# SumitTarafder/Figbird

Hardware: AMD Instinct MI355X
Metric: gaps/sec (+ filled-bases/sec), synthetic 1e5-gap set recipe, jump-library fill pass (higher is better)
Workload: dtype f64

## Files before the change

figbird_amd/api.py:

```python
from __future__ import annotations

import ctypes as C
import os
from dataclasses import dataclass
from dataclasses import replace as dc_replace
from typing import List, Optional

import numpy as np

from . import build as _build

c_double_p = C.POINTER(C.c_double)
c_i32_p = C.POINTER(C.c_int32)
c_i64_p = C.POINTER(C.c_int64)
c_u8_p = C.POINTER(C.c_uint8)


class FigModel(C.Structure):
    _fields_ = [
        ("max_read_length", C.c_int32), ("error_pos_dist", c_double_p), ("in_pos_dist", c_double_p),
        ("del_pos_dist", c_double_p), ("error_type_probs", C.c_double * 25),
        ("insert_len_dist_smoothed", c_double_p), ("max_insert_size", C.c_int32),
        ("insert_threshold_min", C.c_int32), ("insert_threshold_max", C.c_int32), ("gap_prob_cutoff", C.c_int32),
        ("partial_flag", C.c_int32), ("unmapped_flag", C.c_int32), ("script_itr", C.c_int32),
# ... 42 lines not shown

class FigReadPlacement(C.Structure):
    _fields_ = [("ll_drawn", c_double_p), ("ll_other", c_double_p), ("sum_other", c_double_p), ("off_other", c_i32_p), ("n_valid", c_i32_p),
                ("pq", c_u8_p), ("state", c_u8_p)]


PLACE_OFF, PLACE_ON, PLACE_NONE, PLACE_MAX_PQ = 0, 1, 255, 60


@dataclass
class Placement:
    ll_drawn: np.ndarray
    ll_other: np.ndarray
    sum_other: np.ndarray
    off_other: np.ndarray
    n_valid: np.ndarray
    pq: np.ndarray
    state: np.ndarray


class FigStats(C.Structure):
    _fields_ = [("kernel_ms", C.c_double), ("h2d_ms", C.c_double), ("d2h_ms", C.c_double),
                ("packed_bytes", C.c_int64), ("place_calls", C.c_int64), ("alg_flops", C.c_double),
                ("n_launches", C.c_int32), ("pad0", C.c_int32), ("spec_flops", C.c_double),
                ("mle_alg_flops", C.c_double), ("mle_exec_flops", C.c_double)]


EXPORTS = ["fig_version", "fig_strerror", "fig_ctx_create", "fig_ctx_destroy", "fig_ctx_set_model",
           "fig_results_capacity", "fig_batch_upload", "fig_fill_resident", "fig_fill_resident_ex", "fig_batch_free", "fig_fill_gaps",
           "fig_get_stats", "fig_batch_probe_reach", "fig_batch_set_ot_preset", "fig_batch_quality", "fig_batch_placement"]

_lib = None
_host = None


def load_library(path: Optional[str] = None) -> C.CDLL:
    global _lib
    if _lib is not None and path is None:
        return _lib
    p = path or _build.LIB
    if not os.path.exists(p):
        raise RuntimeError(f"libfighip.so not built at {p}: run `python -m figbird_amd.build` (there is no CPU fallback)")
    lib = C.CDLL(p)
    lib.fig_version.restype = C.c_int
    lib.fig_strerror.restype = C.c_char_p
    lib.fig_strerror.argtypes = [C.c_int]
    lib.fig_ctx_create.argtypes = [C.c_int, C.POINTER(C.c_void_p)]
# ... 474 lines not shown
```

figbird_amd/csrc/fig_abi.hip:

```cpp
#include <hip/hip_runtime.h>

#include <algorithm>
#include <cstdio>
#include <cstdlib>
#include <cstring>
#include <new>
#include <vector>
#include <chrono>
#include <thread>
#include <mutex>

#include "../../include/figbird_hip.h"
#include "fig_engine.h"
#include "fig_pack.h"
#include "fig_abi_host.h"
#include "fig_quality.h"
#include "fig_quality_host.h"
#include "fig_placement.h"

#ifdef FIG_PROF
#define FIG_PROF_BEGIN() const unsigned long long _k0 = __builtin_readcyclecounter()
#define FIG_PROF_FLUSH() do { if (E.lane == 0) { atomicAdd(&B.counters[FIG_CNT_WAIT], E.wait_cycles); atomicAdd(&B.counters[FIG_CNT_WAVE], (unsigned long long)__builtin_readcyclecounter() - _k0); \
    for (int i = 0; i < FIG_PROF_SLOTS; i++) if (E.prof[i]) atomicAdd(&B.counters[i < FIG_PROF_SPLIT ? FIG_CNT_PROF_LO + i : FIG_CNT_PROF_HI + (i - FIG_PROF_SPLIT)], E.prof[i]); } } while (0)
#else
// ... 49 lines not shown
    FigEng E; FigScr work;
    fig_kernel_begin(E, M, B, A, LDS_TAB, work);
    FIG_PROF_BEGIN();
    fig_pop_loop(E, B, A, [&] { return fig_src_order(B, A); }, [&](int gi) { fig_item_fill<LDS_TAB>(E, work, gi); });
    FIG_PROF_FLUSH();
    fig_kernel_flush(E, B);
}

template <bool LDS_TAB, int NT>
__global__ void __launch_bounds__(NT, (NT <= 256 ? 2 : 1)) fig_begin_kernel(FigDevModel M, FigDevBatch B, FigKernArgs A) {
    FigEng E; FigScr work;
    fig_kernel_begin(E, M, B, A, LDS_TAB, work);
    fig_pop_loop(E, B, A, [&] { return fig_src_order(B, A); }, [&](int gi) { fig_item_begin<LDS_TAB>(E, work, gi); });
    fig_kernel_flush(E, B);
}

template <bool LDS_TAB, int NT>
__global__ void __launch_bounds__(NT, (NT <= 256 ? 2 : 1)) fig_probe_kernel(FigDevModel M, FigDevBatch B, FigKernArgs A) {
    FigEng E; FigScr work;
    fig_kernel_begin(E, M, B, A, LDS_TAB, work);
    fig_pop_loop(E, B, A, [&] { return fig_src_order(B, A); }, [&](int gi) { fig_item_probe<LDS_TAB>(E, work, gi); });
}

static_assert(sizeof(FigItem) == sizeof(int4) && sizeof(FigEntry) == sizeof(int4), "item records travel as int4");
template <bool LDS_TAB, int NT>
__global__ void __launch_bounds__(NT, (NT <= 256 ? 2 : 1)) fig_eval_kernel(FigDevModel M, FigDevBatch B, FigKernArgs A, const int4 *items, int n_items) {
    FigEng E; FigScr work;
    fig_kernel_begin(E, M, B, A, LDS_TAB, work);
    FIG_PROF_BEGIN();
    fig_pop_loop(E, B, A, [&] { return FigItemSrc<FigItem>{(const FigItem *)items, 0, n_items}; }, [&](FigItem it) { fig_item_eval<LDS_TAB>(E, work, it); });
    FIG_PROF_FLUSH();
    fig_kernel_flush(E, B);
}

__global__ void __launch_bounds__(64) fig_replay_kernel(FigDevModel M, FigDevBatch B, const int4 *entries, int n) {
    if ((int)blockIdx.x >= n) return;
    FigEng E{}; FigScr work{};
    fig_eng_ident(E, threadIdx.x, blockDim.x, 64);
    E.M = &M; E.B = &B; E.nteams = 1; E.S = (FigState *)fig_lds;
    const FigEntry en = ((const FigEntry *)entries)[blockIdx.x];
    fig_item_replay(E, work, en);
}

template <bool LDS_TAB, int NT>
__global__ void __launch_bounds__(NT, (NT <= 256 ? 2 : 1)) fig_end_kernel(FigDevModel M, FigDevBatch B, FigKernArgs A, const int *list, int n) {
    FigEng E; FigScr work;
    fig_kernel_begin(E, M, B, A, LDS_TAB, work);
    fig_pop_loop(E, B, A, [&] { return FigItemSrc<int>{list, 0, n}; }, [&](int gi) { fig_item_end<LDS_TAB>(E, work, gi); });
    fig_kernel_flush(E, B);
}

__global__ void __launch_bounds__(256) fig_stream_kernel(FigDevModel M, FigDevBatch B, uint32_t *out) {
    for (long long gi = blockIdx.x; gi < B.n_gaps; gi += gridDim.x) {
        const FigDevGap &g = B.gaps[gi];
        const int L = M.L;
        const long long n = (long long)((g.nU + FIG_SH_C - 1) / FIG_SH_C) * L * (FIG_SH_C / 2);
        for (long long i = threadIdx.x; i < n; i += blockDim.x) {
            const int sp = (int)(i % (FIG_SH_C / 2));
            const long long cj = i / (FIG_SH_C / 2);
            const int j = (int)(cj % L);
            uint32_t v = 0;
            for (int h = 0; h < 2; h++) {
                const long long r = (cj / L) * FIG_SH_C + 2 * sp + h;
// ... 4 lines not shown
                    if (len == L && !(aux & 2)) {
                        const uint32_t w = B.packed[B.u.woff[idx] + (j >> 4)];
                        e = 0x1000u | (2u * (4u * (unsigned)(aux & 1) + ((w >> ((j & 15) * 2)) & 3u)));
                    }
                }
                v |= e << (16 * h);
            }
            out[g.streamOff + i] = v;
        }
    }
}

#define FIG_HIP(call) do { hipError_t _e = (call); if (_e != hipSuccess) { ctx->last_hip = (int)_e; return FIG_EHIP; } } while (0)

struct DevBuf { void *p = nullptr; };

struct FigTmpBufs {
    std::vector<void *> bufs;
    ~FigTmpBufs() { for (void *p : bufs) hipFree(p); }
    void *alloc(size_t n) { void *p = nullptr; if (hipMalloc(&p, n ? n : 8) != hipSuccess) return nullptr; bufs.push_back(p); return p; }
};

struct FigLane { hipStream_t stream = nullptr; hipEvent_t done = nullptr; int32_t *queue_head = nullptr; uint8_t *scratch = nullptr; FigItem *d_items = nullptr; FigEntry *d_entries = nullptr; size_t cap = 0;
                 FigGapCtl *h_ctl = nullptr; FigItem *h_items = nullptr; FigEntry *h_entries = nullptr; int qsel = 0; };

struct fig_ctx {
    int device = 0;
    hipStream_t stream = nullptr;
    hipEvent_t ev0 = nullptr, ev1 = nullptr;
    int n_cu = 0;
    int last_hip = 0;
    bool have_model = false;
    FigDevModel dm;
    DevBuf d_model_tabs;
    fig_model hm;
    bool have_batch = false;
    FigDevBatch db;
    std::vector<int32_t> h_order;
    struct Cls { FigLaunchClass c; int blocks; int capacity; };
    std::vector<Cls> classes;
    std::vector<DevBuf> bufs;
    int64_t n_gaps = 0, n_ureads = 0, n_preads = 0, str_total = 0;
    std::vector<int64_t> h_str_off;
    int nslots = 32;
    std::vector<FigLane> lanes;
    fig_stats stats;
    int sh_on = FIG_SH_SC;
    std::vector<uint8_t> h_ot;
    uint8_t *d_ot = nullptr;
};

static int dev_alloc(fig_ctx *ctx, size_t bytes, void **out) {
    DevBuf b;
    if (bytes == 0) bytes = 8;
    hipError_t e = hipMalloc(&b.p, bytes);
    if (e != hipSuccess) { ctx->last_hip = (int)e; return FIG_ENOMEM; }
    ctx->bufs.push_back(b);
    *out = b.p;
    return FIG_OK;
}

template <typename T>
static int dev_upload(fig_ctx *ctx, const std::vector<T> &v, const T **out) {
    void *p = nullptr;
    int rc = dev_alloc(ctx, v.size() * sizeof(T), &p);
    if (rc) return rc;
    if (!v.empty()) {
        hipError_t e = hipMemcpyAsync(p, v.data(), v.size() * sizeof(T), hipMemcpyHostToDevice, ctx->stream);
        if (e != hipSuccess) { ctx->last_hip = (int)e; return FIG_EHIP; }
    }
// ... 71 lines not shown
    if (hipMemcpy(ctx->d_model_tabs.p, all.data(), all.size() * sizeof(double), hipMemcpyHostToDevice) != hipSuccess) return FIG_EHIP;
    fig_model_point(ctx->dm, o, (const double *)ctx->d_model_tabs.p);
    ctx->have_model = true;
    return FIG_OK;
}

extern "C" int64_t fig_results_capacity(const fig_model *m, const fig_gap_batch *b) {
    if (!m || !b) return FIG_EINVAL;
    return fig_pack_results_capacity(m, b);
}

enum FigKind { FIG_K_FILL, FIG_K_BEGIN, FIG_K_EVAL, FIG_K_END, FIG_K_PROBE };

template <typename... P, typename... Args>
static hipError_t launch_one(void (*k)(P...), size_t lds, int nt, int blocks, hipStream_t stream, Args... args) {
    hipError_t e = hipFuncSetAttribute((const void *)k, hipFuncAttributeMaxDynamicSharedMemorySize, (int)lds);
    if (e != hipSuccess) return e;
    hipLaunchKernelGGL(k, dim3(blocks), dim3(nt), lds, stream, args...);
    return hipGetLastError();
}

template <bool LDS_TAB, int NT>
static hipError_t launch_kind(fig_ctx *ctx, const fig_ctx::Cls &c, const FigDevBatch &db, hipStream_t stream, FigKind kind, int blocks, const void *list, int n, int qsel) {
    const FigKernArgs A = fig_kargs_of(c.c, qsel, ctx->sh_on);
    switch (kind) {
        case FIG_K_FILL: return launch_one(fig_fill_kernel<LDS_TAB, NT>, c.c.lds, NT, blocks, stream, ctx->dm, db, A);
        case FIG_K_BEGIN: return launch_one(fig_begin_kernel<LDS_TAB, NT>, c.c.lds, NT, blocks, stream, ctx->dm, db, A);
        case FIG_K_PROBE: return launch_one(fig_probe_kernel<LDS_TAB, NT>, c.c.lds, NT, blocks, stream, ctx->dm, db, A);
        case FIG_K_EVAL: return launch_one(fig_eval_kernel<LDS_TAB, NT>, c.c.lds, NT, blocks, stream, ctx->dm, db, A, (const int4 *)list, n);
        case FIG_K_END: return launch_one(fig_end_kernel<LDS_TAB, NT>, c.c.lds, NT, blocks, stream, ctx->dm, db, A, (const int *)list, n);
    }
    return hipErrorInvalidValue;
}

static hipError_t launch_any(fig_ctx *ctx, const fig_ctx::Cls &c, const FigDevBatch &db, hipStream_t stream, FigKind kind, int blocks, const void *list, int n, int qsel = 0) {
    if (c.c.tiles > 0) return launch_kind<true, 512>(ctx, c, db, stream, kind, blocks, list, n, qsel);
    if (c.c.lds_tab) return c.c.nt == 256 ? launch_kind<true, 256>(ctx, c, db, stream, kind, blocks, list, n, qsel) : launch_kind<true, 512>(ctx, c, db, stream, kind, blocks, list, n, qsel);
    return launch_kind<false, 512>(ctx, c, db, stream, kind, blocks, list, n, qsel);
}

extern "C" int fig_batch_upload(fig_ctx *ctx, const fig_gap_batch *b) {
    if (!ctx || !b) return FIG_EINVAL;
    if (!ctx->have_model) return FIG_EINVAL;
    hipSetDevice(ctx->device);
    free_batch(ctx);
    const fig_model *m = &ctx->hm;
    hipEventRecord(ctx->ev0, ctx->stream);
// ... 30 lines not shown
    UP(p_pos, p.pos); UP(p_aux, p.aux); UP(p_clip, p.clip); UP(p_ref, p.refpos); UP(p_len, p.len); UP(p_woff, p.woff); UP(p_qoff, p.qoff);
#undef UP
    db.u.clip = nullptr; db.u.refpos = nullptr; db.u.qoff = nullptr;
    void *p;
    if (m->unmapped_flag) {
        if ((rc = dev_alloc(ctx, (size_t)K.stream_total * 4, &p))) return rc;
        db.ustream = (const uint32_t *)p;
        FIG_HIP(hipMemsetD32Async((hipDeviceptr_t)p, (int)(((0x1000u | FIG_SH_ONE) << 16) | (0x1000u | FIG_SH_ONE)), (size_t)K.stream_total, ctx->stream));
        if (ng > 0) {
            hipLaunchKernelGGL(fig_stream_kernel, dim3((unsigned)std::min<int64_t>(ng, 4096)), dim3(256), 0, ctx->stream, ctx->dm, db, (uint32_t *)p);
            FIG_HIP(hipGetLastError());
        }
    }
    if ((rc = dev_alloc(ctx, (size_t)ng * 4, &p))) return rc; db.filled_len = (int32_t *)p;
    if ((rc = dev_alloc(ctx, (size_t)ng * 4, &p))) return rc; db.gaptofill = (int32_t *)p;
    if ((rc = dev_alloc(ctx, (size_t)K.str_total, &p))) return rc; db.str = (char *)p;
    if ((rc = dev_alloc(ctx, 64 * (ctx->classes.size() + 1), &p))) return rc; db.queue_head = (int32_t *)p;
    if ((rc = dev_alloc(ctx, FIG_CNT_N * sizeof(unsigned long long), &p))) return rc; db.counters = (unsigned long long *)p;
    size_t total_blocks = 0;
    for (const fig_ctx::Cls &c : ctx->classes) total_blocks += (size_t)c.capacity;
    if ((rc = dev_alloc(ctx, (size_t)stride * std::max<size_t>(total_blocks, 1), &p))) return rc; db.scratch = (uint8_t *)p;
    if ((rc = dev_alloc(ctx, (size_t)K.persist_total + 256, &p))) return rc; db.persist = (uint8_t *)p;
    if ((rc = dev_alloc(ctx, (size_t)std::max<int64_t>(ng, 1) * sizeof(FigGapCtl), &p))) return rc; db.gapctl = (FigGapCtl *)p;
    if ((rc = dev_alloc(ctx, (size_t)std::max<int64_t>(ng, 1), &p))) return rc; ctx->d_ot = (uint8_t *)p; db.ot_preset = ctx->d_ot;
    ctx->h_ot = K.ot_preset;
    FIG_HIP(hipMemcpyAsync(ctx->d_ot, ctx->h_ot.data(), (size_t)std::max<int64_t>(ng, 1), hipMemcpyHostToDevice, ctx->stream));
    ctx->nslots = K.nslots;
    {   size_t blk = 0;
        for (size_t ci = 0; ci < ctx->classes.size(); ci++) {
            const fig_ctx::Cls &c = ctx->classes[ci];
            ctx->lanes.push_back(FigLane());
            FigLane &l = ctx->lanes.back();
            if (hipStreamCreate(&l.stream) != hipSuccess || hipEventCreateWithFlags(&l.done, hipEventDisableTiming) != hipSuccess) return FIG_EHIP;
            l.queue_head = db.queue_head + 16 * (ci + 1);
            l.scratch = db.scratch + (size_t)stride * blk; blk += (size_t)c.capacity;
            l.cap = (size_t)std::max(c.c.q_end - c.c.q_begin, 1) * (size_t)(K.nslots + 1);
            if ((rc = dev_alloc(ctx, l.cap * sizeof(FigItem), &p))) return rc; l.d_items = (FigItem *)p;
            if ((rc = dev_alloc(ctx, l.cap * sizeof(FigEntry), &p))) return rc; l.d_entries = (FigEntry *)p;
            if (hipHostMalloc((void **)&l.h_ctl, (size_t)std::max<int64_t>(ng, 1) * sizeof(FigGapCtl), hipHostMallocDefault) != hipSuccess) return FIG_ENOMEM;
            if (hipHostMalloc((void **)&l.h_items, l.cap * sizeof(FigItem), hipHostMallocDefault) != hipSuccess) return FIG_ENOMEM;
            if (hipHostMalloc((void **)&l.h_entries, l.cap * sizeof(FigEntry), hipHostMallocDefault) != hipSuccess) return FIG_ENOMEM;
        }
    }
    db.scratch_stride = stride;
    db.capG = K.capG; db.capR = K.capR; db.capP = K.capP; db.capC = K.capC; db.capW = K.capW; db.capE = K.capE;
    db.n_ureads = ctx->n_ureads;
    FIG_HIP(hipMemsetAsync(db.counters, 0, FIG_CNT_N * sizeof(unsigned long long), ctx->stream));
    FIG_HIP(hipMemsetAsync(db.queue_head, 0, 64 * (ctx->classes.size() + 1), ctx->stream));
    hipEventRecord(ctx->ev1, ctx->stream);
    FIG_HIP(hipStreamSynchronize(ctx->stream));
    float ms = 0; hipEventElapsedTime(&ms, ctx->ev0, ctx->ev1);
    ctx->stats.h2d_ms = ms;
    ctx->stats.packed_bytes = K.packed_bytes();
    ctx->have_batch = true;
    if (!K.ot_given && m->partial_flag && ng > 0 && (rc = fig_ot_carry_measured(ctx, ng))) { free_batch(ctx); return rc; }
    return FIG_OK;
}

extern "C" int fig_batch_probe_reach(fig_ctx *ctx, uint8_t *reach) {
    if (!ctx || !reach || !ctx->have_batch) return FIG_EINVAL;
    hipSetDevice(ctx->device);
// ... 6 lines not shown
    for (const fig_ctx::Cls &c : ctx->classes) {
        FIG_HIP(hipMemsetAsync(db.queue_head, 0, 8, ctx->stream));
        FIG_HIP(launch_any(ctx, c, db, ctx->stream, FIG_K_PROBE, c.blocks, nullptr, 0));
    }
    std::vector<FigGapCtl> ctl((size_t)ng);
    FIG_HIP(hipMemcpyAsync(ctl.data(), db.gapctl, (size_t)ng * sizeof(FigGapCtl), hipMemcpyDeviceToHost, ctx->stream));
    FIG_HIP(hipStreamSynchronize(ctx->stream));
    for (int64_t g = 0; g < ng; g++) reach[g] = ctl[g].reach ? 1 : 0;
    return FIG_OK;
}

extern "C" int fig_batch_set_ot_preset(fig_ctx *ctx, const uint8_t *preset) {
    if (!ctx || !preset || !ctx->have_batch) return FIG_EINVAL;
    hipSetDevice(ctx->device);
    const int64_t ng = ctx->n_gaps;
    for (int64_t g = 0; g < ng; g++) ctx->h_ot[(size_t)g] = preset[g] ? 1 : 0;
    if (ng > 0) { FIG_HIP(hipMemcpy(ctx->d_ot, ctx->h_ot.data(), (size_t)ng, hipMemcpyHostToDevice)); }
    return FIG_OK;
}

static int run_class_parallel(fig_ctx *ctx, const fig_ctx::Cls &c, FigLane &ln, const FigKnobs &knobs) {
    FigDevBatch db = ctx->db;
    db.queue_head = ln.queue_head; db.scratch = ln.scratch;
    hipStream_t stream = ln.stream;
    hipSetDevice(ctx->device);
    int nl = 0;
    hipError_t e;
    auto fail = [&](hipError_t er) { ctx->last_hip = (int)er; return -1; };
    const int capacity = std::max(1, c.capacity);
    auto launch = [&](FigKind kind, int n_work, const void *list) {
        hipError_t er = launch_any(ctx, c, db, stream, kind, std::min(capacity, n_work), list, n_work, ln.qsel);
        ln.qsel ^= 1; nl++;
        return er;
    };
    if ((e = launch(FIG_K_BEGIN, c.c.q_end - c.c.q_begin, nullptr)) != hipSuccess) return fail(e);
    FigGapCtl *ctl = ln.h_ctl;
    const size_t ctl_bytes = (size_t)ctx->n_gaps * sizeof(FigGapCtl);
    const std::vector<int> ids(ctx->h_order.begin() + c.c.q_begin, ctx->h_order.begin() + c.c.q_end);
    FigRound R;
    auto now = [] { return std::chrono::duration<double, std::milli>(std::chrono::steady_clock::now().time_since_epoch()).count(); };
    const double t_start = now();
    double t_prev = now(); int round = 0, last_items = 0, last_active = 0, last_chunk = 0, n_active_max = 0;
    while (true) {
        if ((e = hipMemcpyAsync(ctl, db.gapctl, ctl_bytes, hipMemcpyDeviceToHost, stream)) != hipSuccess) return fail(e);
        if ((e = hipStreamSynchronize(stream)) != hipSuccess) return fail(e);
        fig_plan_round(ids, ctl, capacity, c.c.nsplit, ctx->nslots, knobs.minc, knobs.ipw, n_active_max, R);
        if (knobs.log) { double t = now(); fprintf(stderr, "[figsched] capG=%d round %d: active=%d chunk=%d items=%d blocks=%d  %.1f ms\n", c.c.capG, round, last_active, last_chunk, last_items, capacity, t - t_prev); t_prev = t; }
        round++;
        if (R.n_active == 0) break;
        if (ln.cap < R.items.size() || ln.cap < R.entries.size()) return fail(hipErrorOutOfMemory);
        const int n_items = (int)R.items.size(), n_ent = (int)R.entries.size();
        const size_t items_bytes = R.items.size() * sizeof(FigItem), ent_bytes = R.entries.size() * sizeof(FigEntry);
        last_items = n_items; last_active = R.n_active; last_chunk = R.chunk;
        if (n_items > 0) {
            memcpy(ln.h_items, R.items.data(), items_bytes);
            if ((e = hipMemcpyAsync(ln.d_items, ln.h_items, items_bytes, hipMemcpyHostToDevice, stream)) != hipSuccess) return fail(e);
            if ((e = launch(FIG_K_EVAL, n_items, ln.d_items)) != hipSuccess) return fail(e);
        }
        memcpy(ln.h_entries, R.entries.data(), ent_bytes);
        if ((e = hipMemcpyAsync(ln.d_entries, ln.h_entries, ent_bytes, hipMemcpyHostToDevice, stream)) != hipSuccess) return fail(e);
        hipLaunchKernelGGL(fig_replay_kernel, dim3(n_ent), dim3(64), sizeof(FigState) + 64, stream, ctx->dm, db, (const int4 *)ln.d_entries, n_ent);
        if ((e = hipGetLastError()) != hipSuccess) return fail(e);
        nl++;
    }
    std::vector<int> endlist;
    for (int g : ids) if (ctl[g].status == FIG_GAP_LOOP_DONE) endlist.push_back(g);
    if (!endlist.empty()) {
        if ((e = hipStreamSynchronize(stream)) != hipSuccess) return fail(e);
        memcpy(ln.h_items, endlist.data(), endlist.size() * sizeof(int));
        if ((e = hipMemcpyAsync(ln.d_items, ln.h_items, endlist.size() * sizeof(int), hipMemcpyHostToDevice, stream)) != hipSuccess) return fail(e);
        if ((e = launch(FIG_K_END, (int)endlist.size(), ln.d_items)) != hipSuccess) return fail(e);
        if (knobs.log) { const double t0 = now(); hipStreamSynchronize(stream); fprintf(stderr, "[figsched] capG=%d end kernel: %d gaps, %.1f ms (lane done at %.1f ms since its first round)\n", c.c.capG, (int)endlist.size(), now() - t0, now() - t_start); }
    }
    return nl;
}

extern "C" int fig_fill_resident(fig_ctx *ctx, fig_gap_results *out) { return fig_fill_resident_ex(ctx, out, nullptr); }

extern "C" int fig_fill_resident_ex(fig_ctx *ctx, fig_gap_results *out, const fig_gap_support *sup) {
    if (!ctx || !out || !ctx->have_batch) return FIG_EINVAL;
    if (!out->filled_len || !out->gaptofill || !out->str_off || (!out->str && ctx->str_total > 0)) return FIG_EINVAL;
    if (sup && (!sup->counts || !sup->origin)) return FIG_EINVAL;
    hipSetDevice(ctx->device);
    int64_t ng = ctx->n_gaps;
    FigDevBatch &db = ctx->db;
    FigTmpBufs tmp;
    std::vector<int32_t> hsup(sup ? (size_t)ctx->str_total * 5 : 0);
    const std::vector<FigPlane> planes = fig_fill_planes(db, ctx->n_ureads + ctx->n_preads, ctx->str_total, out, sup, hsup.data());
    auto clear = [&](void *p, int v, size_t n) { return n ? hipMemsetAsync(p, v, n, ctx->stream) : hipSuccess; };
    auto fetch = [&](void *dst, const void *src, size_t n) { return n ? hipMemcpyAsync(dst, src, n, hipMemcpyDeviceToHost, ctx->stream) : hipSuccess; };
    for (const FigPlane &pl : planes) {
        if (!(*pl.dev = tmp.alloc(pl.bytes))) return FIG_ENOMEM;
        if (pl.fill >= 0) FIG_HIP(clear(*pl.dev, pl.fill, pl.bytes));
    }
    FIG_HIP(clear(db.counters, 0, FIG_CNT_N * sizeof(unsigned long long)));
    FIG_HIP(clear(db.queue_head, 0, 64 * (ctx->classes.size() + 1)));
    for (auto &l : ctx->lanes) l.qsel = 0;
    FIG_HIP(clear(db.filled_len, 0, (size_t)std::max<int64_t>(ng, 1) * 4));
    FIG_HIP(clear(db.gaptofill, 0, (size_t)std::max<int64_t>(ng, 1) * 4));
    FIG_HIP(clear(db.str, 'N', (size_t)ctx->str_total));
    FIG_HIP(clear(db.gapctl, 0, (size_t)std::max<int64_t>(ng, 1) * sizeof(FigGapCtl)));
    FIG_HIP(hipEventRecord(ctx->ev0, ctx->stream));
    int nl = 0;
    const FigKnobs knobs = fig_knobs_from_env(ctx->dm.unmapped);
    if (knobs.seq) {
        for (const fig_ctx::Cls &c : ctx->classes) {
            FIG_HIP(clear(db.queue_head, 0, 4));
            FIG_HIP(launch_any(ctx, c, db, ctx->stream, FIG_K_FILL, c.blocks, nullptr, 0));
            nl++;
        }
    } else {
        const size_t nc = ctx->classes.size();
        std::vector<int> rcs(nc, 0);
        for (size_t ci = 0; ci < nc; ci++) FIG_HIP(hipStreamWaitEvent(ctx->lanes[ci].stream, ctx->ev0, 0));
        if (nc <= 1 || knobs.lanes_serial) {
            for (size_t ci = 0; ci < nc; ci++) rcs[ci] = run_class_parallel(ctx, ctx->classes[ci], ctx->lanes[ci], knobs);
        } else {
            std::vector<std::thread> th;
            for (size_t ci = 0; ci < nc; ci++) th.emplace_back([&, ci] { rcs[ci] = run_class_parallel(ctx, ctx->classes[ci], ctx->lanes[ci], knobs); });
            for (auto &t : th) t.join();
        }
        for (size_t ci = 0; ci < nc; ci++) {
            if (rcs[ci] < 0) { hipDeviceSynchronize(); return FIG_EHIP; }
            nl += rcs[ci];
            FIG_HIP(hipEventRecord(ctx->lanes[ci].done, ctx->lanes[ci].stream));
            FIG_HIP(hipStreamWaitEvent(ctx->stream, ctx->lanes[ci].done, 0));
        }
// ... 200 lines not shown
```

figbird_amd/csrc/fig_abi_host.h:

```cpp
#ifndef FIG_ABI_HOST_H
#define FIG_ABI_HOST_H
#include <algorithm>
#include <cmath>
#include <cstdlib>
#include <cstring>
#include <vector>
#include "../../include/figbird_hip.h"
#include "fig_types.h"
#include "fig_gaprules.h"

static_assert(FIG_ORG_NONE == FIG_SUP_NONE && FIG_ORG_FINAL == FIG_SUP_FINAL && FIG_ORG_ORIGINAL == FIG_SUP_ORIGINAL && FIG_ORG_TIEBREAK == FIG_SUP_TIEBREAK,
              "the engine's path mask (fig_types.h) is fig_gap_support::origin");

static inline const char *fig_strerror_text(int code) {
    switch (code) {
        case FIG_OK: return "ok";
        case FIG_EINVAL: return "invalid argument";
        case FIG_ENODEV: return "no usable HIP device (libfighip has no CPU path)";
        case FIG_ENOMEM: return "out of memory";
        case FIG_EHIP: return "HIP runtime error";
        case FIG_ENOSPC: return "result string buffer too small";
        case FIG_EUNSUP: return "input outside the supported envelope";
        default: return "unknown error";
    }
// ... 70 lines not shown
        add(db.dbg_n_cand, out->dbg_n_cand, ng * 4, 0);
        add(db.dbg_cand_i, out->dbg_cand_i, nc * 12, -1);
        add(db.dbg_cand_lik, out->dbg_cand_lik, nc * 8, -1);
        if (out->dbg_n_place) add(db.dbg_n_place, out->dbg_n_place, ng * 4, 0);
        if (out->dbg_counts && out->dbg_plane_cols > 0) { db.dbg_plane_cols = out->dbg_plane_cols; add(db.dbg_counts, out->dbg_counts, nc * out->dbg_plane_cols * 5 * 8, 0); }
        if (out->dbg_read_maxlv && out->dbg_plane_reads > 0) { db.dbg_plane_reads = out->dbg_plane_reads; add(db.dbg_read_maxlv, out->dbg_read_maxlv, nc * out->dbg_plane_reads * 8, 0); }
    }
    if (out->draw_pos && out->draw_isz && out->draw_len) {
        add(db.draw_pos, out->draw_pos, nr * 4, -1);
        add(db.draw_isz, out->draw_isz, nr * 4, 0);
        add(db.draw_len, out->draw_len, ng * 8, -1);
    }
    if (sup) {
        add(db.sup_counts, sup_host, (size_t)str_total * 5 * 4, 0);
        add(db.sup_origin, sup->origin, ng * 4, 0);
    }
    return pl;
}

static inline void fig_stats_from_counters(const unsigned long long *cnt, fig_stats &st) {
    st.place_calls = (int64_t)cnt[FIG_CNT_PLACE];
    st.alg_flops = (double)cnt[FIG_CNT_FLOPS]; st.spec_flops = (double)cnt[FIG_CNT_SPEC];
    st.mle_alg_flops = (double)cnt[FIG_CNT_MLE_ALG]; st.mle_exec_flops = (double)cnt[FIG_CNT_MLE_EXEC];
}

static FigKernArgs fig_kargs_of(const FigLaunchClass &c, int qsel, int sh_on) {
    FigKernArgs A;
    A.capG = c.capG; A.capGl = c.capGl; A.ncolE = c.ncolE; A.Wcap = c.Wcap; A.nteams = c.nteams;
    A.q_begin = c.q_begin; A.q_end = c.q_end; A.qsel = qsel;
    A.tiles = c.tiles; A.tile_step = c.tile_step; A.tile_cols = c.tile_cols; A.tiled_max = c.tiled_max;
    A.sh_on = sh_on;
    return A;
}

static int fig_ot_carry_measured(fig_ctx *ctx, int64_t ng) {
    std::vector<uint8_t> reach((size_t)ng, 0), preset((size_t)ng, 0);
    int rc;
    if ((rc = fig_batch_probe_reach(ctx, reach.data()))) return rc;
    std::vector<int64_t> ids((size_t)ng);
    for (int64_t g = 0; g < ng; g++) ids[(size_t)g] = g;
    fig_ot_carry(ids, reach.data(), preset.data());
    return fig_batch_set_ot_preset(ctx, preset.data());
}

static int fig_compact_results(int64_t ng, const char *src, const int64_t *src_off, fig_gap_results *out) {
    int64_t need = 0;
// ... 6 lines not shown
        if (n > 0) { memcpy(out->str + o, src + src_off[g], (size_t)n); o += n; }
    }
    out->str_off[ng] = o;
    return FIG_OK;
}

static void fig_compact_support(int64_t ng, const int32_t *src, const int64_t *src_off, const fig_gap_results *out, int32_t *dst) {
    for (int64_t g = 0; g < ng; g++) {
        int n = out->filled_len[g];
        if (n > 0) memcpy(dst + out->str_off[g] * 5, src + src_off[g] * 5, (size_t)n * 5 * sizeof(int32_t));
    }
}

static int fig_fill_gaps_once(fig_ctx *ctx, const fig_gap_batch *batch, fig_gap_results *out) {
    int rc = fig_batch_upload(ctx, batch);
    if (rc) return rc;
    rc = fig_fill_resident(ctx, out);
    fig_batch_free(ctx);
    return rc;
}

struct FigKnobs {
    bool seq;
    bool lanes_serial;
    bool log;
    int minc;
    double ipw;
    int sh_on;
};

static FigKnobs fig_knobs_from_env(int unmapped) {
    FigKnobs k;
    const char *sched = getenv("FIG_SCHED"), *ser = getenv("FIG_LANES"), *mc = getenv("FIG_MIN_CHUNK"), *ipw = getenv("FIG_ITEMS_PER_WG");
    const char *ev = getenv("FIG_ESTEP"), *sc = getenv("FIG_SH_CHUNKS");
    k.seq = sched && strcmp(sched, "seq") == 0;
    k.lanes_serial = ser && strcmp(ser, "serial") == 0;
    k.log = getenv("FIG_SCHED_LOG") != nullptr;
    k.minc = mc ? std::max(1, atoi(mc)) : 16;
    k.ipw = ipw ? std::max(1.0, atof(ipw)) : (unmapped ? 12.0 : 6.0);
    k.sh_on = (ev && !strcmp(ev, "pair")) ? 0 : (sc ? std::max(1, std::min(FIG_SH_SC, atoi(sc))) : FIG_SH_SC);
    return k;
}

struct FigRound { std::vector<FigItem> items; std::vector<FigEntry> entries; int chunk = 0, n_active = 0; };

static void fig_plan_round(const std::vector<int> &ids, const FigGapCtl *ctl, int capacity, int nsplit, int slots_cap, int minc, double ipw_base,
                           int &n_active_max, FigRound &R) {
    R.items.clear(); R.entries.clear();
    R.chunk = 0; R.n_active = 0;
    for (int g : ids) if (ctl[g].status == FIG_GAP_MORE) R.n_active++;
    if (R.n_active == 0) return;
    long long rem_total = 0;
    for (int g : ids) if (ctl[g].status == FIG_GAP_MORE) rem_total += std::max(0, ctl[g].range - ctl[g].j);
    n_active_max = std::max(n_active_max, R.n_active);
    const double ipw = ipw_base * std::min(8.0, std::max(1.0, n_active_max / 96.0));
    const double share = rem_total > 0 ? (ipw * capacity / (double)std::max(1, nsplit)) / (double)rem_total : 1.0;
    const double target = ipw * capacity / (double)std::max(1, nsplit);
    long long total = 0;
    for (int g : ids) {
        if (ctl[g].status != FIG_GAP_MORE) continue;
        if ((double)total >= 1.25 * target) break;
        int j = ctl[g].j, range = ctl[g].range;
        int want = (int)std::ceil((range - j) * share);
        want = std::min(std::max(want, minc), slots_cap);
        int n = std::max(0, std::min(want, range - j));
        R.chunk = std::max(R.chunk, n);
        total += n;
        R.entries.push_back(FigEntry{g, n, 0, 0});
    }
    for (const FigEntry &en : R.entries)
        for (int k = en.n - 1; k >= 0; k--) R.items.push_back(FigItem{en.gap, ctl[en.gap].j + k, k, 0});
}

#endif
```

figbird_amd/csrc/fig_engine.h:

```cpp
#ifndef FIG_ENGINE_H
#define FIG_ENGINE_H

#include "fig_types.h"

#ifdef FIG_EMU
#include <cmath>
#include <cstring>
#define FIG_D static inline
#define FIG_NOINLINE
#define FIG_HD static inline
#define FIG_SYNC() ((void)0)
FIG_D double fig_log10(double x) { return log10(x); }
FIG_D double fig_log(double x) { return log(x); }
FIG_D double fig_exp(double x) { return exp(x); }
FIG_D double fig_pow10(double x) { return pow(10, x); }
FIG_D int fig_atomic_add_i32(int *p, int v) { int o = *p; *p += v; return o; }
FIG_D void fig_atomic_max_i32(int *p, int v) { if (v > *p) *p = v; }
FIG_D int fig_atomic_fetch_add_i32(int *p, int v) { int o = *p; *p += v; return o; }
FIG_D void fig_atomic_min_i32(int *p, int v) { if (v < *p) *p = v; }
FIG_D void fig_atomic_or_i32(int *p, int v) { *p |= v; }
FIG_D void fig_atomic_add_u64(unsigned long long *p, unsigned long long v) { *p += v; }
FIG_D unsigned long long fig_shfl_down_u64(unsigned long long v, int off) { (void)v; (void)off; return 0; }
#else
#include <hip/hip_runtime.h>
// ... 198 lines not shown
    int tiles, tile_step, tile_cols;
    double *wbuf;
    int Wcap, nteams;
    int sh_on;
    int lane, wave, nw, wsz;
    const double *kt_fwd, *kt_rev;
    const double *mt_fwd, *mt_rev;
    unsigned char *rb;
    uint32_t *plb;
    unsigned char *gs;
    int capG;
    unsigned long long flops;
    unsigned long long mle_alg;
    unsigned long long mle_exec;
    unsigned long long wait_cycles;
    unsigned long long prof[FIG_PROF_SLOTS];
};

FIG_D void fig_eng_ident(FigEng &E, unsigned tid, unsigned nt, unsigned wsz) {
    E.tid = (int)tid; E.nt = (int)nt;
    E.lane = (int)(tid % wsz); E.wave = (int)(tid / wsz); E.nw = (int)((nt + wsz - 1) / wsz); E.wsz = (int)wsz;
}

struct FigKernArgs { int capG, capGl, ncolE, Wcap, nteams, q_begin, q_end, qsel, tiles, tile_step, tile_cols, tiled_max, sh_on; };

FIG_D long long fig_eng_carve(FigEng &E, const FigDevModel &M, const FigKernArgs &A, bool lds_tab) {
    E.capG = A.capG;
    E.ncolE = A.ncolE; E.xoff = M.L - 1; E.Wcap = A.Wcap; E.nteams = A.nteams; E.sh_on = A.sh_on;
    long long off = 0;
    E.pq_lds = lds_tab; E.w_lds = lds_tab;
    E.tiles = A.tiles; E.tile_step = A.tile_step; E.tile_cols = A.tile_cols;
    if (lds_tab && A.tiles > 0) {
        E.pq_lds = 0;
        E.off_pq = 0; E.off_q4 = 8 * A.tile_cols; E.off_w = 9 * A.tile_cols;
        off = 9LL * A.tile_cols + (long long)A.nteams * A.Wcap;
        { const long long mle = FIG_TILED_MLE_DOUBLES(A.ncolE, (int)E.nw); if (mle > off && mle <= A.tiled_max) off = mle; }
        E.pq = E.scr.pqg; E.q4 = E.scr.q4g; E.wbuf = E.scr.wg;
    } else if (lds_tab) {
        E.off_pq = 0; E.off_q4 = 8 * A.ncolE; E.off_w = 9 * A.ncolE;
        off = 9LL * A.ncolE + (long long)A.nteams * A.Wcap;
        E.pq = (FigPQ *)(fig_lds + E.off_pq); E.q4 = fig_lds + E.off_q4; E.wbuf = fig_lds + E.off_w;
    } else {
        E.off_pq = E.off_q4 = E.off_w = 0;
        E.pq = E.scr.pqg; E.q4 = E.scr.q4g; E.wbuf = E.scr.wg;
    }
    E.S = (FigState *)(fig_lds + off); E.lds_tw = (int)off;
    unsigned char *bp = (unsigned char *)(E.S + 1);
// ... 331 lines not shown
```

figbird_amd/csrc/fig_engine_sched.h:

```cpp
#ifndef FIG_ENGINE_SCHED_H
#define FIG_ENGINE_SCHED_H

template <bool LDS>
FIG_D void fig_gap_begin(FigEng &E) {
    FigState &S = *E.S;
    const FigDevModel &M = *E.M;
    const FigDevGap &g = *E.g;
    int G0 = g.G0, nU = g.nU;
    if (E.tid == 0) {
        S.left = M.D; S.right = M.D; S.side_limit = 30; S.end_pos_max = 0;
        S.valid_count = S.invalid_count = 0;
        S.partial_read_count = M.partial_flag == 1 ? g.nP : 0;
        S.region_perct = 0; S.region_perct_max = 0;
        S.partial_read_len = M.partial_len;
        S.rep_flag = 0; S.one_side_repeat_flag = 0; S.large_gap_flag = g.lgf; S.comp_count = 0;
        S.left_max = 0; S.right_min = 0; S.discont_or_not = 0;
        S.psr_temp[0] = S.psr_temp[1] = S.psr_final[0] = S.psr_final[1] = -1;
        S.umaxleftf = S.umaxrightf = S.ucoverf = 0;
        S.num_itr = 0; S.overlap_threshold = (E.B->ot_preset && E.B->ot_preset[g.gapNo]) ? 5 : 0; S.gaptofill = 0;
        S.gl_len = S.gr_len = S.pl_len = S.pr_len = 0;
        S.cons_len = 1; E.scr.cons[0] = 4;
        E.scr.used_read_arr[0] = 0;
        S.best_len = S.cur_len = S.prev_len = S.orig_len = 0;
        S.flops_useful = 0; S.n_place = 0; S.dbg_j = -1; S.sup_origin = FIG_ORG_NONE;
// ... 460 lines not shown
template <bool LDS>
FIG_D void fig_item_eval(FigEng &E, const FigScr &work, const FigItem &it) {
    E.g = &E.B->gaps[it.gap];
    FigPersist P; fig_persist_of(*E.B, *E.g, P);
    fig_spec_eval<LDS>(E, work, P, it.j, it.slot, E.g->capGg);
    FIG_SYNC();
}

FIG_D void fig_item_replay(FigEng &E, const FigScr &work, const FigEntry &en) {
    E.g = &E.B->gaps[en.gap];
    FigPersist P; fig_persist_of(*E.B, *E.g, P);
    fig_spec_replay(E, work, P, en.n, E.g->capGg);
    fig_ctl_publish(E, en.gap);
}

template <bool LDS>
FIG_D void fig_item_end(FigEng &E, const FigScr &work, int gi) {
    FigPersist P; fig_item_gap(E, work, gi, P);
    fig_state_load(E, P);
    fig_gap_end<LDS>(E);
    if (E.tid == 0) fig_ctl_of(E, gi).status = FIG_GAP_FINISHED;
    FIG_SYNC();
}
#endif
```

figbird_amd/csrc/fig_types.h:

```cpp
#ifndef FIG_TYPES_H
#define FIG_TYPES_H
#include <stdint.h>

#define FIG_MAX_READLEN 200
#define FIG_READ_CAP 3000
#define FIG_MAX_GAP 100000
#define FIG_FLANK 208
#define FIG_DBL_MAX 1.7976931348623157e308
#define FIG_SH_C 32
#define FIG_SH_SC 4
#define FIG_SH_ONE 16
#define FIG_MLE_FB 208
#define FIG_TILED_MLE_DOUBLES(ncolE, nw) (7LL * (ncolE) + (long long)(nw) * FIG_MLE_FB + ((ncolE) + 15) / 16 + 16 + 8)

enum { FIG_ORG_NONE = 0, FIG_ORG_FINAL = 1, FIG_ORG_ORIGINAL = 2, FIG_ORG_TIEBREAK = 4 };

enum { FIG_GAP_FINISHED = 0, FIG_GAP_MORE = 1, FIG_GAP_LOOP_DONE = 2 };
struct FigGapCtl { int32_t status, j, range, reach; };

struct alignas(16) FigItem { int32_t gap, j, slot, pad; };
struct alignas(16) FigEntry { int32_t gap, n, pad0, pad1; };
static_assert(sizeof(FigGapCtl) == 16 && sizeof(FigItem) == 16 && sizeof(FigEntry) == 16, "control words are four int32: buffers and copies are sized by sizeof");

enum FigCounter {
    FIG_CNT_PLACE = 0,
    FIG_CNT_FLOPS = 1, FIG_CNT_SPEC = 2,
    FIG_CNT_MLE_ALG = 3, FIG_CNT_MLE_EXEC = 4,
    FIG_CNT_PROF_LO = 8, FIG_CNT_WAIT = 30, FIG_CNT_WAVE = 31, FIG_CNT_PROF_HI = 32,
    FIG_CNT_N = 64
};
#define FIG_PROF_SLOTS 40
#define FIG_PROF_SPLIT 22

struct FigDevModel {
    int32_t L;
    int32_t Tmin, Tmax, cutoff;
    int32_t partial_flag, unmapped, script_itr, D, read_length, neg_overlap, partial_len, unm_limit;
    int32_t max_insert;
    double T[25];
    const double *e;
    const double *ome;
    const double *ome1;
    const double *m3;
    const double *insd;
    const double *qtab;
    double fmm_up;
};

struct FigDevGap {
    int64_t gapStart, contigLen;
// ... 19 lines not shown
    const int64_t *qoff;
};

struct FigDevBatch {
    int64_t n_gaps;
    const FigDevGap *gaps;
    const int32_t *order;
    FigDevReads u, p;
    const uint32_t *packed;
    const uint32_t *ustream;
    const uint8_t *qual;
    const uint8_t *flank;
    int32_t *filled_len, *gaptofill; char *str;
    int32_t dbg_max_cand; int32_t *dbg_n_cand; int32_t *dbg_cand_i; double *dbg_cand_lik; int32_t *dbg_n_place;
    int32_t *draw_pos, *draw_isz, *draw_len; int64_t n_ureads;
    int32_t dbg_plane_cols, dbg_plane_reads; double *dbg_counts, *dbg_read_maxlv;
    int32_t *queue_head;
    unsigned long long *counters;
    uint8_t *scratch; int64_t scratch_stride;
    int32_t capG, capR, capP, capC;
    int32_t capW, capE;
    uint8_t *persist;
    FigGapCtl *gapctl;
    const uint8_t *ot_preset;
    int32_t *sup_counts, *sup_origin;
};

#endif
```

include/figbird_hip.h:

```cpp
#ifndef FIGBIRD_HIP_H
#define FIGBIRD_HIP_H

#include <stdint.h>

#ifdef __cplusplus
extern "C" {
#endif

#define FIG_ABI_VERSION 1

#define FIG_OK 0
#define FIG_EINVAL (-1)
#define FIG_ENODEV (-2)
#define FIG_ENOMEM (-3)
#define FIG_EHIP (-4)
#define FIG_ENOSPC (-5)
#define FIG_EUNSUP (-6)

typedef struct fig_ctx fig_ctx;

typedef struct fig_model {
    int32_t max_read_length;
    const double *error_pos_dist;
    const double *in_pos_dist;
// ... 78 lines not shown
} fig_gap_quality;

#define FIG_PLACE_OFF 0
#define FIG_PLACE_ON  1
#define FIG_PLACE_NONE 255
#define FIG_PLACE_MAX_PQ 60
typedef struct fig_read_placement {
    double  *ll_drawn;
    double  *ll_other;
    double  *sum_other;
    int32_t *off_other;
    int32_t *n_valid;
    uint8_t *pq;
    uint8_t *state;
} fig_read_placement;

typedef struct fig_stats {
    double kernel_ms;
    double h2d_ms, d2h_ms;
    int64_t packed_bytes;
    int64_t place_calls;
    double alg_flops;
    int32_t n_launches;
    int32_t pad0;
    double spec_flops;
    double mle_alg_flops;
    double mle_exec_flops;
} fig_stats;

int fig_version(void);
const char *fig_strerror(int code);

int fig_ctx_create(int device_ordinal, fig_ctx **out);
void fig_ctx_destroy(fig_ctx *ctx);
int fig_ctx_set_model(fig_ctx *ctx, const fig_model *model);

int64_t fig_results_capacity(const fig_model *model, const fig_gap_batch *batch);

int fig_batch_upload(fig_ctx *ctx, const fig_gap_batch *batch);
int fig_fill_resident(fig_ctx *ctx, fig_gap_results *out);
int fig_fill_resident_ex(fig_ctx *ctx, fig_gap_results *out, const fig_gap_support *sup);
void fig_batch_free(fig_ctx *ctx);
int fig_fill_gaps(fig_ctx *ctx, const fig_gap_batch *batch, fig_gap_results *out);

int fig_batch_probe_reach(fig_ctx *ctx, uint8_t *reach);
int fig_batch_set_ot_preset(fig_ctx *ctx, const uint8_t *preset);

// ... 11 lines not shown
```

Before: 23.96.

## Add in-kernel continuation queue so eval kernel chains gap chunks without host rounds

Adds a device-side continuation scheduler. The workgroup that finishes the last chunk of a gap replays it, then publishes the next chunk or end item to a global queue, and resident workgroups pop and run those entries inside the same eval launch. It aims to remove per-round host round-trips, replay launches and the tail idle time between rounds. In exchange it adds atomics, fences and a linear scan over the queue on every pop. It is enabled by default only when the unmapped flag is set or FIG_SCHED=continuous, so whether the benchmark uses it depends on its model.

New measurement: 24.60 (median of 6 runs). 2.7% higher.

```diff
diff --git a/figbird_amd/api.py b/figbird_amd/api.py
--- a/figbird_amd/api.py
+++ b/figbird_amd/api.py
@@ -88,7 +88,7 @@
 class FigStats(C.Structure):
     _fields_ = [("kernel_ms", C.c_double), ("h2d_ms", C.c_double), ("d2h_ms", C.c_double),
                 ("packed_bytes", C.c_int64), ("place_calls", C.c_int64), ("alg_flops", C.c_double),
-                ("n_launches", C.c_int32), ("pad0", C.c_int32), ("spec_flops", C.c_double),
+                ("n_launches", C.c_int32), ("cont_chunks", C.c_int32), ("spec_flops", C.c_double),
                 ("mle_alg_flops", C.c_double), ("mle_exec_flops", C.c_double)]
 
 
diff --git a/figbird_amd/csrc/fig_abi.hip b/figbird_amd/csrc/fig_abi.hip
--- a/figbird_amd/csrc/fig_abi.hip
+++ b/figbird_amd/csrc/fig_abi.hip
@@ -95,13 +95,101 @@
     fig_pop_loop(E, B, A, [&] { return fig_src_order(B, A); }, [&](int gi) { fig_item_probe<LDS_TAB>(E, work, gi); });
 }
 
+FIG_D int fig_ld_acquire(const int32_t *p) { return __hip_atomic_load(p, __ATOMIC_ACQUIRE, __HIP_MEMORY_SCOPE_AGENT); }
+FIG_D int fig_ld_relaxed(const int32_t *p) { return __hip_atomic_load(p, __ATOMIC_RELAXED, __HIP_MEMORY_SCOPE_AGENT); }
+
+FIG_D bool fig_chunk_finished(FigEng &E, const FigDevBatch &B, int gi, int n) {
+    __threadfence();
+    __syncthreads();
+    if (E.tid == 0) {
+        const int done = __hip_atomic_fetch_add(B.gap_pending + gi, 1, __ATOMIC_ACQ_REL, __HIP_MEMORY_SCOPE_AGENT) + 1;
+        if (done == n) __hip_atomic_store(B.gap_pending + gi, 0, __ATOMIC_RELAXED, __HIP_MEMORY_SCOPE_AGENT);
+        E.S->bc_i = done == n;
+    }
+    __syncthreads();
+    const bool last = E.S->bc_i != 0;
+    __syncthreads();
+    if (last) __threadfence();
+    return last;
+}
+
+FIG_D void fig_cont_publish(FigEng &E, const FigDevBatch &B, const FigKernArgs &A, const FigCont &c) {
+    __threadfence();
+    __syncthreads();
+    if (E.tid == 0) {
+        bool ok = true;
+        if (c.kind == FIG_CONT_EVAL) {
+            const long long live = (long long)gridDim.x - fig_ld_relaxed(&B.cont_hdr->exited);
+            ok = live * 100 >= (long long)c.n * A.cont_live;
+        }
+        if (ok) {
+            const int idx = atomicAdd(&B.cont_hdr->tail, 1);
+            if (idx < B.cont_cap) {
+                FigCont *e = B.cont + idx;
+                e->gap = c.gap; e->j0 = c.j0; e->n = c.n; e->kind = c.kind; e->next = 0; e->rank = c.rank; e->pad = 0;
+                __hip_atomic_store(&e->ready, 1, __ATOMIC_RELEASE, __HIP_MEMORY_SCOPE_AGENT);
+                if (c.kind == FIG_CONT_EVAL) atomicAdd(&B.counters[FIG_CNT_CONT], 1ull);
+            }
+        }
+    }
+    __syncthreads();
+}
+
+FIG_D bool fig_cont_pop(FigEng &E, const FigDevBatch &B, const FigKernArgs &A, FigCont &out, int &k) {
+    FigState &S = *E.S;
+    if (E.tid == 0) { const int t = fig_ld_relaxed(&B.cont_hdr->tail); S.bc_j = t < B.cont_cap ? t : B.cont_cap; }
+    __syncthreads();
+    const int tail = S.bc_j;
+    __syncthreads();
+    for (int pass = 0; pass <= tail; pass++) {
+        if (E.tid == 0) S.bc_i = -1;
+        __syncthreads();
+        int best = -1;
+        for (int i = E.tid; i < tail; i += E.nt) {
+            const FigCont *e = B.cont + i;
+            if (!fig_ld_acquire(&e->ready)) continue;
+            if (fig_ld_relaxed(&e->next) >= e->n) continue;
+            const int rank = A.cont_prio ? (e->rank < 32767 ? e->rank : 32767) : 0;
+            const int key = rank * 65536 + (FIG_CONT_CAP_MAX - i);
+            best = key > best ? key : best;
+        }
+        if (best >= 0) atomicMax(&S.bc_i, best);
+        __syncthreads();
+        const int key = S.bc_i;
+        if (key < 0) { __syncthreads(); return false; }
+        const int idx = FIG_CONT_CAP_MAX - (key & 65535);
+        if (E.tid == 0) S.bc_j = atomicAdd(&B.cont[idx].next, 1);
+        __syncthreads();
+        k = S.bc_j;
+        __syncthreads();
+        if (k < B.cont[idx].n) { __threadfence(); out = B.cont[idx]; return true; }
+    }
+    return false;
+}
+
 static_assert(sizeof(FigItem) == sizeof(int4) && sizeof(FigEntry) == sizeof(int4), "item records travel as int4");
 template <bool LDS_TAB, int NT>
 __global__ void __launch_bounds__(NT, (NT <= 256 ? 2 : 1)) fig_eval_kernel(FigDevModel M, FigDevBatch B, FigKernArgs A, const int4 *items, int n_items) {
     FigEng E; FigScr work;
     fig_kernel_begin(E, M, B, A, LDS_TAB, work);
     FIG_PROF_BEGIN();
-    fig_pop_loop(E, B, A, [&] { return FigItemSrc<FigItem>{(const FigItem *)items, 0, n_items}; }, [&](FigItem it) { fig_item_eval<LDS_TAB>(E, work, it); });
+    auto eval = [&](FigItem it) {
+        fig_item_eval<LDS_TAB>(E, work, it);
+        if (A.cont && it.chunk > 0 && fig_chunk_finished(E, B, it.gap, it.chunk)) {
+            FigCont nx;
+            fig_item_continue(E, work, it.gap, it.chunk, A.minc, nx);
+            fig_cont_publish(E, B, A, nx);
+        }
+    };
+    fig_pop_loop(E, B, A, [&] { return FigItemSrc<FigItem>{(const FigItem *)items, 0, n_items}; }, eval);
+    if (A.cont) {
+        FigCont c; int k;
+        while (fig_cont_pop(E, B, A, c, k)) {
+            if (c.kind == FIG_CONT_END) fig_item_end<LDS_TAB>(E, work, c.gap);
+            else eval(FigItem{c.gap, c.j0 + k, k, c.n});
+        }
+        if (E.tid == 0) atomicAdd(&B.cont_hdr->exited, 1);
+    }
     FIG_PROF_FLUSH();
     fig_kernel_flush(E, B);
 }
@@ -112,6 +200,10 @@
     fig_eng_ident(E, threadIdx.x, blockDim.x, 64);
     E.M = &M; E.B = &B; E.nteams = 1; E.S = (FigState *)fig_lds;
     const FigEntry en = ((const FigEntry *)entries)[blockIdx.x];
+    if (en.stamped) {
+        const FigGapCtl c = B.gapctl[en.gap];
+        if (c.status != FIG_GAP_MORE || c.j != en.j_planned || en.n != 0) return;
+    }
     fig_item_replay(E, work, en);
 }
 
@@ -162,7 +254,8 @@
 };
 
 struct FigLane { hipStream_t stream = nullptr; hipEvent_t done = nullptr; int32_t *queue_head = nullptr; uint8_t *scratch = nullptr; FigItem *d_items = nullptr; FigEntry *d_entries = nullptr; size_t cap = 0;
-                 FigGapCtl *h_ctl = nullptr; FigItem *h_items = nullptr; FigEntry *h_entries = nullptr; int qsel = 0; };
+                 FigGapCtl *h_ctl = nullptr; FigItem *h_items = nullptr; FigEntry *h_entries = nullptr; int qsel = 0;
+                 uint8_t *d_cont = nullptr; int cont_cap = 0; };
 
 struct fig_ctx {
     int device = 0;
@@ -186,6 +279,7 @@
     std::vector<FigLane> lanes;
     fig_stats stats;
     int sh_on = FIG_SH_SC;
+    FigKnobs fill_knobs;
     std::vector<uint8_t> h_ot;
     uint8_t *d_ot = nullptr;
 };
@@ -303,7 +397,8 @@
 
 template <bool LDS_TAB, int NT>
 static hipError_t launch_kind(fig_ctx *ctx, const fig_ctx::Cls &c, const FigDevBatch &db, hipStream_t stream, FigKind kind, int blocks, const void *list, int n, int qsel) {
-    const FigKernArgs A = fig_kargs_of(c.c, qsel, ctx->sh_on);
+    FigKernArgs A = fig_kargs_of(c.c, qsel, ctx->sh_on);
+    if (kind == FIG_K_EVAL) { const FigKnobs &kn = ctx->fill_knobs; A.cont = kn.cont && db.cont_cap > 0; A.minc = kn.minc; A.cont_live = kn.cont_live; A.cont_prio = kn.cont_prio; }
     switch (kind) {
         case FIG_K_FILL: return launch_one(fig_fill_kernel<LDS_TAB, NT>, c.c.lds, NT, blocks, stream, ctx->dm, db, A);
         case FIG_K_BEGIN: return launch_one(fig_begin_kernel<LDS_TAB, NT>, c.c.lds, NT, blocks, stream, ctx->dm, db, A);
@@ -380,6 +475,7 @@
     if ((rc = dev_alloc(ctx, (size_t)stride * std::max<size_t>(total_blocks, 1), &p))) return rc; db.scratch = (uint8_t *)p;
     if ((rc = dev_alloc(ctx, (size_t)K.persist_total + 256, &p))) return rc; db.persist = (uint8_t *)p;
     if ((rc = dev_alloc(ctx, (size_t)std::max<int64_t>(ng, 1) * sizeof(FigGapCtl), &p))) return rc; db.gapctl = (FigGapCtl *)p;
+    if ((rc = dev_alloc(ctx, (size_t)std::max<int64_t>(ng, 1) * 4, &p))) return rc; db.gap_pending = (int32_t *)p;
     if ((rc = dev_alloc(ctx, (size_t)std::max<int64_t>(ng, 1), &p))) return rc; ctx->d_ot = (uint8_t *)p; db.ot_preset = ctx->d_ot;
     ctx->h_ot = K.ot_preset;
     FIG_HIP(hipMemcpyAsync(ctx->d_ot, ctx->h_ot.data(), (size_t)std::max<int64_t>(ng, 1), hipMemcpyHostToDevice, ctx->stream));
@@ -395,6 +491,8 @@
             l.cap = (size_t)std::max(c.c.q_end - c.c.q_begin, 1) * (size_t)(K.nslots + 1);
             if ((rc = dev_alloc(ctx, l.cap * sizeof(FigItem), &p))) return rc; l.d_items = (FigItem *)p;
             if ((rc = dev_alloc(ctx, l.cap * sizeof(FigEntry), &p))) return rc; l.d_entries = (FigEntry *)p;
+            l.cont_cap = fig_cont_capacity(std::vector<int>(K.order.begin() + c.c.q_begin, K.order.begin() + c.c.q_end), K.gaps, fig_knobs_from_env(0).minc);
+            if ((rc = dev_alloc(ctx, sizeof(FigContHdr) + (size_t)l.cont_cap * sizeof(FigCont), &p))) return rc; l.d_cont = (uint8_t *)p;
             if (hipHostMalloc((void **)&l.h_ctl, (size_t)std::max<int64_t>(ng, 1) * sizeof(FigGapCtl), hipHostMallocDefault) != hipSuccess) return FIG_ENOMEM;
             if (hipHostMalloc((void **)&l.h_items, l.cap * sizeof(FigItem), hipHostMallocDefault) != hipSuccess) return FIG_ENOMEM;
             if (hipHostMalloc((void **)&l.h_entries, l.cap * sizeof(FigEntry), hipHostMallocDefault) != hipSuccess) return FIG_ENOMEM;
@@ -447,6 +545,9 @@
 static int run_class_parallel(fig_ctx *ctx, const fig_ctx::Cls &c, FigLane &ln, const FigKnobs &knobs) {
     FigDevBatch db = ctx->db;
     db.queue_head = ln.queue_head; db.scratch = ln.scratch;
+    db.cont_hdr = (FigContHdr *)ln.d_cont; db.cont = (FigCont *)(ln.d_cont + sizeof(FigContHdr));
+    db.cont_cap = knobs.cont ? std::min(ln.cont_cap, knobs.cont_cap) : 0;
+    const size_t cont_bytes = sizeof(FigContHdr) + (size_t)db.cont_cap * sizeof(FigCont);
     hipStream_t stream = ln.stream;
     hipSetDevice(ctx->device);
     int nl = 0;
@@ -474,14 +575,17 @@
         round++;
         if (R.n_active == 0) break;
         if (ln.cap < R.items.size() || ln.cap < R.entries.size()) return fail(hipErrorOutOfMemory);
+        const int n_empty = knobs.cont ? fig_round_stamp(R, ctl) : 0;
         const int n_items = (int)R.items.size(), n_ent = (int)R.entries.size();
         const size_t items_bytes = R.items.size() * sizeof(FigItem), ent_bytes = R.entries.size() * sizeof(FigEntry);
         last_items = n_items; last_active = R.n_active; last_chunk = R.chunk;
         if (n_items > 0) {
             memcpy(ln.h_items, R.items.data(), items_bytes);
             if ((e = hipMemcpyAsync(ln.d_items, ln.h_items, items_bytes, hipMemcpyHostToDevice, stream)) != hipSuccess) return fail(e);
+            if (knobs.cont && (e = hipMemsetAsync(ln.d_cont, 0, cont_bytes, stream)) != hipSuccess) return fail(e);
             if ((e = launch(FIG_K_EVAL, n_items, ln.d_items)) != hipSuccess) return fail(e);
         }
+        if (knobs.cont && n_empty == 0) continue;
         memcpy(ln.h_entries, R.entries.data(), ent_bytes);
         if ((e = hipMemcpyAsync(ln.d_entries, ln.h_entries, ent_bytes, hipMemcpyHostToDevice, stream)) != hipSuccess) return fail(e);
         hipLaunchKernelGGL(fig_replay_kernel, dim3(n_ent), dim3(64), sizeof(FigState) + 64, stream, ctx->dm, db, (const int4 *)ln.d_entries, n_ent);
@@ -525,9 +629,11 @@
     FIG_HIP(clear(db.gaptofill, 0, (size_t)std::max<int64_t>(ng, 1) * 4));
     FIG_HIP(clear(db.str, 'N', (size_t)ctx->str_total));
     FIG_HIP(clear(db.gapctl, 0, (size_t)std::max<int64_t>(ng, 1) * sizeof(FigGapCtl)));
+    FIG_HIP(clear(db.gap_pending, 0, (size_t)std::max<int64_t>(ng, 1) * 4));
     FIG_HIP(hipEventRecord(ctx->ev0, ctx->stream));
     int nl = 0;
     const FigKnobs knobs = fig_knobs_from_env(ctx->dm.unmapped);
+    ctx->fill_knobs = knobs;
     if (knobs.seq) {
         for (const fig_ctx::Cls &c : ctx->classes) {
             FIG_HIP(clear(db.queue_head, 0, 4));
diff --git a/figbird_amd/csrc/fig_abi_host.h b/figbird_amd/csrc/fig_abi_host.h
--- a/figbird_amd/csrc/fig_abi_host.h
+++ b/figbird_amd/csrc/fig_abi_host.h
@@ -116,6 +116,7 @@
     st.place_calls = (int64_t)cnt[FIG_CNT_PLACE];
     st.alg_flops = (double)cnt[FIG_CNT_FLOPS]; st.spec_flops = (double)cnt[FIG_CNT_SPEC];
     st.mle_alg_flops = (double)cnt[FIG_CNT_MLE_ALG]; st.mle_exec_flops = (double)cnt[FIG_CNT_MLE_EXEC];
+    st.cont_chunks = (int32_t)cnt[FIG_CNT_CONT];
 }
 
 static FigKernArgs fig_kargs_of(const FigLaunchClass &c, int qsel, int sh_on) {
@@ -168,6 +169,7 @@
 
 struct FigKnobs {
     bool seq;
+    bool cont; int cont_cap, cont_live, cont_prio;
     bool lanes_serial;
     bool log;
     int minc;
@@ -180,6 +182,11 @@
     const char *sched = getenv("FIG_SCHED"), *ser = getenv("FIG_LANES"), *mc = getenv("FIG_MIN_CHUNK"), *ipw = getenv("FIG_ITEMS_PER_WG");
     const char *ev = getenv("FIG_ESTEP"), *sc = getenv("FIG_SH_CHUNKS");
     k.seq = sched && strcmp(sched, "seq") == 0;
+    const char *cc = getenv("FIG_CONT_CAP"), *cl = getenv("FIG_CONT_LIVE"), *cp = getenv("FIG_CONT_PRIO");
+    k.cont = sched ? strcmp(sched, "continuous") == 0 : unmapped != 0;
+    k.cont_cap = cc ? std::max(1, atoi(cc)) : FIG_CONT_CAP_MAX;
+    k.cont_live = cl ? std::max(0, atoi(cl)) : 100;
+    k.cont_prio = cp ? (atoi(cp) != 0) : 1;
     k.lanes_serial = ser && strcmp(ser, "serial") == 0;
     k.log = getenv("FIG_SCHED_LOG") != nullptr;
     k.minc = mc ? std::max(1, atoi(mc)) : 16;
@@ -218,4 +225,20 @@
         for (int k = en.n - 1; k >= 0; k--) R.items.push_back(FigItem{en.gap, ctl[en.gap].j + k, k, 0});
 }
 
+static int fig_round_stamp(FigRound &R, const FigGapCtl *ctl) {
+    size_t pos = 0; int n_empty = 0;
+    for (FigEntry &en : R.entries) {
+        en.j_planned = ctl[en.gap].j; en.stamped = 1;
+        if (en.n == 0) n_empty++;
+        for (int k = 0; k < en.n; k++) R.items[pos++].chunk = en.n;
+    }
+    return n_empty;
+}
+
+static int fig_cont_capacity(const std::vector<int> &ids, const std::vector<FigDevGap> &gaps, int minc) {
+    long long n = 0;
+    for (int g : ids) n += gaps[(size_t)g].rangeCap / std::max(1, minc) + 3;
+    return (int)std::min<long long>(std::max<long long>(n, 1), FIG_CONT_CAP_MAX);
+}
+
 #endif
diff --git a/figbird_amd/csrc/fig_engine.h b/figbird_amd/csrc/fig_engine.h
--- a/figbird_amd/csrc/fig_engine.h
+++ b/figbird_amd/csrc/fig_engine.h
@@ -244,7 +244,8 @@
     E.lane = (int)(tid % wsz); E.wave = (int)(tid / wsz); E.nw = (int)((nt + wsz - 1) / wsz); E.wsz = (int)wsz;
 }
 
-struct FigKernArgs { int capG, capGl, ncolE, Wcap, nteams, q_begin, q_end, qsel, tiles, tile_step, tile_cols, tiled_max, sh_on; };
+struct FigKernArgs { int capG, capGl, ncolE, Wcap, nteams, q_begin, q_end, qsel, tiles, tile_step, tile_cols, tiled_max, sh_on;
+                     int cont = 0, minc = 16, cont_live = 100, cont_prio = 1; };
 
 FIG_D long long fig_eng_carve(FigEng &E, const FigDevModel &M, const FigKernArgs &A, bool lds_tab) {
     E.capG = A.capG;
diff --git a/figbird_amd/csrc/fig_engine_sched.h b/figbird_amd/csrc/fig_engine_sched.h
--- a/figbird_amd/csrc/fig_engine_sched.h
+++ b/figbird_amd/csrc/fig_engine_sched.h
@@ -506,4 +506,26 @@
     if (E.tid == 0) fig_ctl_of(E, gi).status = FIG_GAP_FINISHED;
     FIG_SYNC();
 }
+
+
+FIG_HD int fig_cont_chunk(int minc, int last, int slots, int left) {
+    int n = last > minc ? last : minc;
+    if (n > slots) n = slots;
+    if (n > left) n = left;
+    return n;
+}
+
+FIG_D void fig_item_continue(FigEng &E, const FigScr &work, int gi, int n, int minc, FigCont &next) {
+    fig_item_replay(E, work, FigEntry{gi, n, 0, 0});
+    FIG_SYNC();
+    const FigLoop &L = E.S->L;
+    next.gap = gi; next.next = 0; next.ready = 0; next.pad = 0;
+    if (L.done) { next.kind = FIG_CONT_END; next.j0 = 0; next.n = 1; next.rank = 1; }
+    else {
+        const int left = L.range - L.j;
+        next.kind = FIG_CONT_EVAL; next.j0 = L.j; next.n = fig_cont_chunk(minc, n, E.g->nslots, left);
+        next.rank = (left + next.n - 1) / (next.n > 0 ? next.n : 1);
+    }
+    FIG_SYNC();
+}
 #endif
diff --git a/figbird_amd/csrc/fig_types.h b/figbird_amd/csrc/fig_types.h
--- a/figbird_amd/csrc/fig_types.h
+++ b/figbird_amd/csrc/fig_types.h
@@ -18,14 +18,20 @@
 enum { FIG_GAP_FINISHED = 0, FIG_GAP_MORE = 1, FIG_GAP_LOOP_DONE = 2 };
 struct FigGapCtl { int32_t status, j, range, reach; };
 
-struct alignas(16) FigItem { int32_t gap, j, slot, pad; };
-struct alignas(16) FigEntry { int32_t gap, n, pad0, pad1; };
+struct alignas(16) FigItem { int32_t gap, j, slot, chunk; };
+struct alignas(16) FigEntry { int32_t gap, n, j_planned, stamped; };
 static_assert(sizeof(FigGapCtl) == 16 && sizeof(FigItem) == 16 && sizeof(FigEntry) == 16, "control words are four int32: buffers and copies are sized by sizeof");
+enum { FIG_CONT_EVAL = 0, FIG_CONT_END = 1 };
+#define FIG_CONT_CAP_MAX 65535
+struct alignas(16) FigCont { int32_t gap, j0, n, kind; int32_t next, ready, rank, pad; };
+struct alignas(16) FigContHdr { int32_t tail, exited, pad[2]; };
+static_assert(sizeof(FigCont) == 32 && sizeof(FigContHdr) == 16, "continuation records: buffers are sized by sizeof");
 
 enum FigCounter {
     FIG_CNT_PLACE = 0,
     FIG_CNT_FLOPS = 1, FIG_CNT_SPEC = 2,
     FIG_CNT_MLE_ALG = 3, FIG_CNT_MLE_EXEC = 4,
+    FIG_CNT_CONT = 5,
     FIG_CNT_PROF_LO = 8, FIG_CNT_WAIT = 30, FIG_CNT_WAVE = 31, FIG_CNT_PROF_HI = 32,
     FIG_CNT_N = 64
 };
@@ -91,6 +97,7 @@
     int32_t capW, capE;
     uint8_t *persist;
     FigGapCtl *gapctl;
+    int32_t *gap_pending; FigContHdr *cont_hdr; FigCont *cont; int32_t cont_cap;
     const uint8_t *ot_preset;
     int32_t *sup_counts, *sup_origin;
 };
diff --git a/include/figbird_hip.h b/include/figbird_hip.h
--- a/include/figbird_hip.h
+++ b/include/figbird_hip.h
@@ -124,7 +124,7 @@
     int64_t place_calls;
     double alg_flops;
     int32_t n_launches;
-    int32_t pad0;
+    int32_t cont_chunks;
     double spec_flops;
     double mle_alg_flops;
     double mle_exec_flops;
```
